# cahekp/Raymarching

Hardware: AMD Instinct MI355X
Metric: ray-steps/sec + frames/sec at 4096×4096, 1/2/4/8 MI355X (higher is better)
Workload: dtype f32; 1 GPU; C3: 4096x4096 scene T (template.frag), 256 max steps, pose P0, row bands of 16 over 1 GPU(s), rgba8 frame on rank 0; scene=T, W=4096, H=4096, max_steps=256, pose=P0, band=16, fmt=rgba8, wire=rgba8, streams=1, kernel=auto, chunks=1, schedule=adaptive, ray_steps_per_frame=1074511601, executed_ray_steps_per_frame=398047527

## Files before the change

include/rm.h:

```cpp
#ifndef RM_H_
#define RM_H_

#include <stddef.h>
#include <stdint.h>

#ifdef __cplusplus
extern "C" {
#endif

#define RM_ABI_VERSION 3

typedef enum rm_status {
    RM_OK = 0,
    RM_ERR_INVALID_ARGUMENT = 1,
    RM_ERR_FILE = 2,
    RM_ERR_SCENE = 3,
    RM_ERR_NO_SCENE = 4,
    RM_ERR_DEVICE = 5,
    RM_ERR_OUT_OF_MEMORY = 6
} rm_status;

typedef struct rm_ctx rm_ctx;

typedef struct rm_params {
// ... 170 lines not shown
    RM_TONEMAP_REINHARD = 2,
    RM_TONEMAP_REINHARD_JODIE = 3,
    RM_TONEMAP_UNCHARTED2 = 4
} rm_tonemap;

rm_status rm_post_frag(rm_ctx *ctx, int W, int H, int sample, int tonemap, const uint32_t *in, uint32_t *out);

rm_status rm_post_chain_ex(rm_ctx *ctx, int W, int H, int sample, int tonemap, const uint32_t *in, uint32_t *mid,
                           uint32_t *out);

rm_status rm_resolution_cache_info(rm_ctx *ctx, int *entries, int *capacity);

rm_status rm_certified_steps(rm_ctx *ctx, uint64_t *steps);

rm_status rm_reflection_cleared_steps(rm_ctx *ctx, uint64_t *steps);

const char *rm_render_code_hash(void);

rm_status rm_cycle_rows(int H, int cycle, int offset, int run, int *nrows);
rm_status rm_render_cycle_rows(rm_ctx *ctx, int W, int H, int cycle, int offset, int run, int row_begin,
                               int row_count, float *out, rm_stats *stats);
rm_status rm_render_cycle_rows_rgba8(rm_ctx *ctx, int W, int H, int cycle, int offset, int run, int row_begin,
                                     int row_count, uint32_t *out, rm_stats *stats);
rm_status rm_deinterleave_cycle_rgb8(rm_ctx *ctx, int W, int H, int cycle, int nparts, const int *offsets,
                                     const int *runs, const int64_t *part_bytes, const uint8_t *gathered,
                                     uint32_t *out);

int64_t rm_wire_capacity(int W, int nrows);
int64_t rm_wire_workspace_bytes(int W, int nrows);
rm_status rm_wire_encode(rm_ctx *ctx, int W, int nrows, const uint32_t *rows, uint8_t *msg, void *workspace,
// ... 41 lines not shown
```

raymarching_amd/_lib.py:

```python
from __future__ import annotations

import ctypes
import os

HERE = os.path.dirname(os.path.abspath(__file__))
LIB_PATH = os.environ.get("RM_LIB") or os.path.join(HERE, "librm.so")

RM_OK = 0
STATUS = {0: "RM_OK", 1: "RM_ERR_INVALID_ARGUMENT", 2: "RM_ERR_FILE", 3: "RM_ERR_SCENE",
          4: "RM_ERR_NO_SCENE", 5: "RM_ERR_DEVICE", 6: "RM_ERR_OUT_OF_MEMORY"}
STATUS_CODES = {v: k for k, v in STATUS.items()}

EXPORTS = ("rm_create", "rm_destroy", "rm_load_scene", "rm_set_uniform1f", "rm_set_uniform2f",
           "rm_set_uniform3f", "rm_set_params", "rm_get_params", "rm_set_stream", "rm_set_stream_kept",
           "rm_synchronize",
           "rm_render", "rm_render_band", "rm_render_rows", "rm_shard_rows", "rm_deinterleave", "rm_deinterleave_rgba8",
           "rm_pack_rgba8", "rm_pack_rgb8", "rm_deinterleave_rgb8",
           "rm_render_rgba8", "rm_render_accumulate", "rm_render_accumulate_rgba8", "rm_render_band_rgba8", "rm_render_rows_rgba8", "rm_fxaa", "rm_bloom", "rm_post_chain", "rm_post_frag", "rm_post_chain_ex",
           "rm_render_code_hash", "rm_render_cycle_rows_wire", "rm_last_error", "rm_status_string",
           "rm_compile_scene", "rm_scene_eval", "rm_render_step_map", "rm_sharded_layout", "rm_comm_get_id",
           "rm_comm_init_rank", "rm_comm_init_all", "rm_comm_destroy", "rm_render_sharded", "rm_render_sharded_all",
           "rm_set_tile_order", "rm_tile_grid", "rm_comm_info", "rm_abi_version", "rm_cycle_rows",
           "rm_render_cycle_rows", "rm_render_cycle_rows_rgba8", "rm_deinterleave_cycle_rgb8",
           "rm_render_sharded_runs", "rm_render_sharded_runs_all", "rm_wire_capacity", "rm_wire_workspace_bytes",
           "rm_wire_encode", "rm_wire_decode", "rm_scatter_part_rgba8", "rm_wire_decode_parts",
           "rm_set_uniform4f", "rm_set_uniform1i", "rm_set_uniformfv", "rm_uniform_count", "rm_uniform_info_at",
           "rm_get_uniformfv", "rm_get_uniform1i", "rm_cast_rays", "rm_camera_rays",
           "rm_aa_offsets", "rm_aa_edge_mask", "rm_refine_rgba8", "rm_render_aa_rgba8", "rm_shade_rays", "rm_scene_eval_form",
           "rm_resolution_cache_info", "rm_certified_steps", "rm_reflection_cleared_steps",
           "rm_batch_bytes", "rm_render_batch", "rm_render_batch_rgba8")

ABI_VERSION = 3
DISPATCH = {0: "row-major", 1: "explicit", 2: "adaptive"}
POST_SAMPLES = {"fxaa": 0, "texel": 1, "chromatic": 2}
TONEMAPS = {"none": 0, "aces": 1, "reinhard": 2, "jodie": 3, "uncharted2": 4}


class RmParams(ctypes.Structure):
    _fields_ = [("max_steps", ctypes.c_int32), ("shadow_max_steps", ctypes.c_int32),
                ("count_evals", ctypes.c_int32), ("kernel", ctypes.c_int32), ("schedule", ctypes.c_int32)]


class RmStats(ctypes.Structure):
    _fields_ = [("evals", ctypes.c_uint64), ("pixels", ctypes.c_uint64), ("kernel_ms", ctypes.c_float),
# ... 143 lines not shown
        "rm_sharded_layout": ([c.c_int, c.c_int, c.c_int, c.c_int, c.c_int, c.POINTER(RmShardLayout)], c.c_int),
        "rm_comm_get_id": ([c.POINTER(RmCommId)], c.c_int),
        "rm_comm_init_rank": ([c.POINTER(vp), vp, c.c_int, c.POINTER(RmCommId), c.c_int], c.c_int),
        "rm_comm_init_all": ([c.POINTER(vp), c.POINTER(vp), c.c_int], c.c_int),
        "rm_comm_destroy": ([vp], c.c_int),
        "rm_comm_info": ([vp, c.POINTER(c.c_int), c.POINTER(c.c_int), c.POINTER(c.c_int)], c.c_int),
        "rm_render_sharded": ([vp, c.c_int, c.c_int, c.c_int, vp, c.POINTER(RmStats)], c.c_int),
        "rm_render_sharded_all": ([c.POINTER(vp), c.c_int, c.c_int, c.c_int, c.c_int, vp, c.POINTER(RmStats)],
                                  c.c_int),
        "rm_set_tile_order": ([vp, vp, c.c_int64], c.c_int),
        "rm_tile_grid": ([c.POINTER(RmParams), c.c_int, c.c_int, c.POINTER(c.c_int), c.POINTER(c.c_int)], c.c_int),
        "rm_abi_version": ([], c.c_int),
        "rm_resolution_cache_info": ([vp, c.POINTER(c.c_int), c.POINTER(c.c_int)], c.c_int),
        "rm_certified_steps": ([vp, c.POINTER(c.c_uint64)], c.c_int),
        "rm_reflection_cleared_steps": ([vp, c.POINTER(c.c_uint64)], c.c_int),
        "rm_cycle_rows": ([c.c_int, c.c_int, c.c_int, c.c_int, c.POINTER(c.c_int)], c.c_int),
        "rm_render_cycle_rows": ([vp, c.c_int, c.c_int, c.c_int, c.c_int, c.c_int, c.c_int, c.c_int, vp,
                                  c.POINTER(RmStats)], c.c_int),
        "rm_render_cycle_rows_rgba8": ([vp, c.c_int, c.c_int, c.c_int, c.c_int, c.c_int, c.c_int, c.c_int, vp,
                                        c.POINTER(RmStats)], c.c_int),
        "rm_deinterleave_cycle_rgb8": ([vp, c.c_int, c.c_int, c.c_int, c.c_int, vp, vp, vp, vp, vp], c.c_int),
        "rm_wire_capacity": ([c.c_int, c.c_int], c.c_int64),
        "rm_wire_workspace_bytes": ([c.c_int, c.c_int], c.c_int64),
        "rm_wire_encode": ([vp, c.c_int, c.c_int, vp, vp, vp, vp], c.c_int),
        "rm_wire_decode": ([vp, c.c_int, c.c_int, c.c_int, c.c_int, c.c_int, c.c_int, vp, vp], c.c_int),
        "rm_scatter_part_rgba8": ([vp, c.c_int, c.c_int, c.c_int, c.c_int, c.c_int, c.c_int, vp, vp], c.c_int),
        "rm_wire_decode_parts": ([vp, c.c_int, c.c_int, c.c_int, c.c_int, vp, vp, vp, vp, vp], c.c_int),
        "rm_render_sharded_runs": ([vp, c.c_int, c.c_int, vp, vp, c.POINTER(RmStats)], c.c_int),
        "rm_render_sharded_runs_all": ([c.POINTER(vp), c.c_int, c.c_int, c.c_int, vp, vp, c.POINTER(RmStats)],
                                       c.c_int),
# ... 19 lines not shown
```

raymarching_amd/api.py:

```python
from __future__ import annotations

import ctypes
import sys

from . import _lib
from ._lib import RmParams, RmStats, check, lib


def _torch():
    import torch
    return torch


class Renderer:

    def __init__(self, device: int = 0):
        L = lib()
        self._ctx = ctypes.c_void_p()
        st = L.rm_create(ctypes.byref(self._ctx), int(device))
        if st != 0:
            raise _lib.RmError(st, f"rm_create(device={device}) failed")
        self.device = int(device)
        self._uniform_types = {}

# ... 123 lines not shown

    @staticmethod
    def _ptr(t):
        return ctypes.c_void_p(t.data_ptr()) if hasattr(t, "data_ptr") else ctypes.c_void_p(t.ctypes.data)

    def certified_steps(self) -> int:
        n = ctypes.c_uint64(0)
        check(lib().rm_certified_steps(self._ctx, ctypes.byref(n)), self._ctx)
        return int(n.value)

    def reflection_cleared_steps(self) -> int:
        n = ctypes.c_uint64(0)
        check(lib().rm_reflection_cleared_steps(self._ctx, ctypes.byref(n)), self._ctx)
        return int(n.value)

    def _stats(self, s) -> dict:
        return dict(s.as_dict(), certified=self.certified_steps(), reflection_cleared=self.reflection_cleared_steps())

    def render(self, W: int, H: int, out=None, stats: bool = False):
        torch = _torch()
        if out is None:
            out = torch.empty((H, W, 4), dtype=torch.float32, device=f"cuda:{self.device}")
        _check_out(out, H * W * 4)
        s = RmStats()
        check(lib().rm_render(self._ctx, int(W), int(H), self._ptr(out), ctypes.byref(s) if stats else None),
              self._ctx)
        return (out, self._stats(s)) if stats else out

    def render_accumulate(self, W: int, H: int, accum, stats: bool = False):
        torch = _torch()
        rgba8 = accum.dtype == torch.int32
        if not rgba8 and accum.dtype != torch.float32:
# ... 635 lines not shown
```

raymarching_amd/csrc/rm_batch_host.cpp:

```cpp
#include <cmath>
#include <cstring>

#include "rm_batch.h"
#include "rm_ctx.h"
#include "rm_trace.h"

using rm::FrameConst;
using rm::RowPart;
using namespace rmhost;

namespace {

int64_t pixel_bytes(bool rgba8) { return rgba8 ? (int64_t)sizeof(uint32_t) : (int64_t)sizeof(float4); }

rm_status batch_host_block(rm_ctx *ctx, size_t bytes, rm_ctx::BatchSlot *&slot) {
    slot = &ctx->batch_slot[ctx->batch_next];
    ctx->batch_next = (ctx->batch_next + 1) % rm_ctx::kBatchSlots;
    if (slot->used) RM_HIP(hipEventSynchronize(slot->copied));
    slot->used = false;
    if (!slot->copied) RM_HIP(hipEventCreateWithFlags(&slot->copied, hipEventDisableTiming));
    if (slot->bytes < bytes) {
        if (slot->host) (void)hipHostFree(slot->host);
        slot->host = nullptr;
        slot->bytes = 0;
// ... 22 lines not shown
    if (rm_status st = frame_rcp(ctx, F)) return st;
    F.row0 = 0;
    F.tile_run = rm::wave_row_mode(part, 0, 8, F.run_magic != 0);
    F.lat_tiles = 0;

    const size_t bytes = (size_t)n * rm::batch_record_bytes(ctx->scene);
    rm_ctx::BatchSlot *slot = nullptr;
    if (rm_status st = batch_host_block(ctx, bytes, slot)) return st;
    FrameConst V = F;
    for (int v = 0; v < n; v++) {
        pose_const(V, views[v].pos, views[v].mouse, views[v].time);
        V.jit_x = seed_jitter(views[v].offset[0] + 0.5f);
        V.jit_y = seed_jitter(views[v].offset[1] + 0.5f);
        rm::batch_record_write(ctx->scene, slot->host, v, V);
    }
    if (rm_status st = batch_scratch(ctx, bytes)) return st;
    void *rec_d = ctx->batch_views;
    RM_HIP(hipMemcpyAsync(rec_d, slot->host, bytes, hipMemcpyHostToDevice, ctx->stream));
    RM_HIP(hipEventRecord(slot->copied, ctx->stream));
    slot->used = true;
    ctx->batch_stream = ctx->stream;
    ctx->batch_pending = true;
    mark_done(ctx);

    ctx->last_certified = 0;
    ctx->last_refl_cleared = 0;
    if (stats) RM_HIP(hipEventRecord(ctx->ev0, ctx->stream));
    const hipError_t e = ctx->scene == rm::SCENE_S0 || ctx->scene == rm::SCENE_T
                             ? rm::launch_batch_t(ctx->scene, F, rec_d, n, out, rgba8, ctx->stream)
                             : rm::launch_batch_o(ctx->scene, F, rec_d, n, out, rgba8, ctx->stream);
    if (e != hipSuccess) return hip_fail(ctx, e, "view batch launch");
    if (stats) {
        RM_HIP(hipEventRecord(ctx->ev1, ctx->stream));
        RM_HIP(hipEventSynchronize(ctx->ev1));
        float ms = 0.0f;
        RM_HIP(hipEventElapsedTime(&ms, ctx->ev0, ctx->ev1));
        std::memset(stats, 0, sizeof(*stats));
        stats->pixels = (uint64_t)n * (uint64_t)W * (uint64_t)H;
        stats->kernel_ms = ms;
        stats->scene = ctx->scene;
        stats->dispatch = RM_DISPATCH_ROW_MAJOR;
// ... 60 lines not shown
```

raymarching_amd/csrc/rm_capi.cpp:

```cpp
#include <cstdio>
#include <cstring>
#include <fstream>
#include <initializer_list>
#include <string>

#include "rm_ctx.h"
#include "rm_internal.h"
#include "rm_scene_file.h"
#include "rm_trace.h"

using rm::cycle_part;
using rm::FrameConst;
using rm::RowPart;
using rm::rows_of_part;
using namespace rmhost;

static_assert(rmscene::kSceneS0 == rm::SCENE_S0 && rmscene::kSceneT == rm::SCENE_T &&
                  rmscene::kSceneO == rm::SCENE_O && rmscene::kSceneOG == rm::SCENE_OG &&
                  rmscene::kScenePlugin == rm::SCENE_PLUGIN,
              "rm_scene_file.h restates rm::SceneId");

namespace {

template <class Launch>
// ... 24 lines not shown
void rm_internal_set_error(rm_ctx *ctx, const std::string &msg) { ctx->err = msg; }

extern "C" {

rm_status rm_create(rm_ctx **out, int device) {
    if (!out) return RM_ERR_INVALID_ARGUMENT;
    *out = nullptr;
    int n = 0;
    if (hipGetDeviceCount(&n) != hipSuccess || device < 0 || device >= n) {
        (void)hipGetLastError();
        return RM_ERR_DEVICE;
    }
    rm_ctx *ctx = new rm_ctx();
    ctx->device = device;
    hipError_t e = hipSetDevice(device);
    if (e == hipSuccess) e = hipMalloc(&ctx->d_evals, 5 * sizeof(unsigned long long));
    if (e == hipSuccess) e = hipEventCreate(&ctx->ev0);
    if (e == hipSuccess) e = hipEventCreate(&ctx->ev1);
    if (e == hipSuccess) e = hipEventCreateWithFlags(&ctx->done, hipEventDisableTiming);
    ctx->persist.reserve(rm_ctx::kPersistBlocks);
    if (e != hipSuccess) {
        rm_destroy(ctx);
        return e == hipErrorOutOfMemory ? RM_ERR_OUT_OF_MEMORY : RM_ERR_DEVICE;
    }
    *out = ctx;
    return RM_OK;
}

rm_status rm_destroy(rm_ctx *ctx) {
    if (!ctx) return RM_ERR_INVALID_ARGUMENT;
    (void)hipSetDevice(ctx->device);
// ... 739 lines not shown

int rm_abi_version(void) { return RM_ABI_VERSION; }

rm_status rm_certified_steps(rm_ctx *ctx, uint64_t *steps) {
    if (!ctx || !steps) return RM_ERR_INVALID_ARGUMENT;
    *steps = ctx->last_certified;
    return RM_OK;
}

rm_status rm_reflection_cleared_steps(rm_ctx *ctx, uint64_t *steps) {
    if (!ctx || !steps) return RM_ERR_INVALID_ARGUMENT;
    *steps = ctx->last_refl_cleared;
    return RM_OK;
}

rm_status rm_resolution_cache_info(rm_ctx *ctx, int *entries, int *capacity) {
    if (!ctx) return RM_ERR_INVALID_ARGUMENT;
    if (entries) *entries = ctx->rcp_n;
    if (capacity) *capacity = rm_ctx::kRcpEntries;
    return RM_OK;
}

const char *rm_last_error(rm_ctx *ctx) { return ctx ? ctx->err.c_str() : "null context"; }

const char *rm_status_string(rm_status s) {
    switch (s) {
    case RM_OK: return "RM_OK";
    case RM_ERR_INVALID_ARGUMENT: return "RM_ERR_INVALID_ARGUMENT";
    case RM_ERR_FILE: return "RM_ERR_FILE";
    case RM_ERR_SCENE: return "RM_ERR_SCENE";
// ... 9 lines not shown
```

raymarching_amd/csrc/rm_ctx.h:

```cpp
#pragma once
#include <hip/hip_runtime.h>

#include <set>
#include <string>
#include <vector>

#include "../../include/rm.h"
#include "rm_launch.h"
#include "rm_plugin_host.h"
#include "rm_rows.h"

struct rm_ctx {
    int device = 0;
    hipStream_t stream = nullptr;
    int scene = -1;
    std::string scene_file;
    float res[2] = {0.0f, 0.0f};
    bool res_set = false;
    float pos[3] = {0.0f, 0.0f, 0.0f};
    float mouse[2] = {0.0f, 0.0f};
    float time = 0.0f;
    struct PersistBlock {
        hipStream_t stream = nullptr;
        uint32_t *ctr = nullptr;
// ... 1 lines not shown
        uint64_t used = 0;
    };
    static constexpr int kPersistBlocks = 4;
    std::vector<PersistBlock> persist;
    hipEvent_t done = nullptr;
    bool dirty = false;
    std::vector<hipEvent_t> retired;
    std::vector<hipStream_t> kept, owed;
    float sample_part = 1.0f;
    float seed1[2] = {0.0f, 0.0f}, seed2[2] = {0.0f, 0.0f};
    rm_params params = {128, 0, 0, 0, 1};
    std::string err;
    std::set<std::string> warned;
    unsigned long long *d_evals = nullptr;
    unsigned long long last_certified = 0;
    unsigned long long last_refl_cleared = 0;
    hipEvent_t ev0 = nullptr, ev1 = nullptr;
    float4 *staging = nullptr;
    size_t staging_bytes = 0;
    uint32_t *mips = nullptr;
    size_t mips_texels = 0;
    int bloom_runs_w = 0, bloom_runs_h = 0;
    hipStream_t bloom_runs_stream = nullptr;
    hipEvent_t bloom_ev = nullptr;
    hipStream_t bloom_stream = nullptr;
    bool bloom_pending = false;
    uint32_t *aa_queue = nullptr;
    size_t aa_words = 0;
    hipEvent_t aa_ev = nullptr;
    hipStream_t aa_stream = nullptr;
// ... 115 lines not shown
```

raymarching_amd/csrc/rm_device.h:

```cpp
#pragma once
#ifdef __HIPCC_RTC__
using __hip_internal::uint32_t;
using __hip_internal::uint64_t;
#else
#include <hip/hip_runtime.h>
#include <stdint.h>
#endif
#include "rm_far_sky.h"
#include "rm_shadow_clear.h"
#include "rm_refl_clear.h"

namespace rm {

enum SceneId : int { SCENE_S0 = 0, SCENE_T = 1, SCENE_O = 2, SCENE_OG = 3, SCENE_PLUGIN = 4 };

constexpr float ZNEAR = 0.02f;
constexpr float ZFAR = 50.0f;
constexpr float PI_REF = 3.1416f;

struct FrameConst {
    float res_x, res_y;
    float pos_x, pos_y, pos_z;
    float cam1_c, cam1_s;
    float cam2_c, cam2_s;
// ... 10 lines not shown
    float sss_floor[2][32];
    uint32_t* evals_map;
    const uint32_t* tile_order;
    uint32_t* tile_cost;
    int lat_tiles;
    int accumulate;
    float sample_part;
    float jit_x, jit_y;
    uint32_t* persist;
    uint32_t run_magic;
    uint32_t gx_magic;
    float camq_x, camq_y, camq_z;
    int far_sky;
    float rcp_w, rcp_h, rcp_res_y;
    int tile_run;
};
static_assert(rmfs::kFarSkyDepth == ZFAR, "rm_far_sky.h restates ZFAR");
static_assert(rmrc::kNear == ZNEAR, "rm_refl_clear.h restates ZNEAR");

__host__ inline void camera_sponge_origin(FrameConst& F) {
    const float x = F.pos_x, y = F.pos_y - 3.0f, z = F.pos_z;
    const float x1 = __builtin_fmaf(x, F.ry_c, z * F.ry_s);
    const float z1 = __builtin_fmaf(z, F.ry_c, -(x * F.ry_s));
    F.camq_x = x1;
    F.camq_y = __builtin_fmaf(y, F.rx_c, -(z1 * F.rx_s));
    F.camq_z = __builtin_fmaf(z1, F.rx_c, y * F.rx_s);
}

__host__ __device__ inline uint32_t div_magic(uint32_t d, uint64_t a_end) {
    return d >= 2 && a_end * (uint64_t)d < (1ull << 32) ? (uint32_t)((1ull << 32) / d + 1) : 0u;
// ... 78 lines not shown
    const float c1 = y2 * (y2 * (y2 * -0.0204391631f + 0.2536086171f) + -1.2336977925f) + 1.0f;
    const float s1 = y * (y2 * (y2 * (y2 * -0.0046075748f + 0.0796819754f) + -0.645963615f) + 1.5707963235f);
    const float c2 = c1 * c1 - s1 * s1;
    const float s2 = 2.0f * s1 * c1;
    return 2.0f * s2 * c2 * (1.0f / (s2 * s2 + c2 * c2));
}
__host__ __device__ inline float glsl_cos(float x) { return glsl_sin(x + 1.57079632f); }


struct Tally {
    uint32_t evals = 0;
    uint32_t flop = 0;
    uint32_t skipped = 0;
    uint32_t certified = 0;
    uint32_t refl_cleared = 0;
};
constexpr uint32_t FL_SPHERE = 9;
constexpr uint32_t FL_TRANSFORM = 18;
constexpr uint32_t FL_LINRAY = 6;
constexpr uint32_t FL_BOX = 17;
constexpr uint32_t FL_FOLD = 40;
constexpr uint32_t FL_CUBE = 21;
constexpr uint32_t FL_SMIN = 12;
constexpr uint32_t FL_BOUNDS = 16;

__device__ __forceinline__ float div_const(float x, float b, float rb) {
    float q = x * rb;
    float r = fmaf(-b, q, x);
    return fmaf(r, rb, q);
}
// ... 299 lines not shown
```

raymarching_amd/csrc/rm_far_sky.h:

```cpp
#pragma once

#if defined(__HIPCC__) || defined(__HIPCC_RTC__) || defined(__HIP__)
#define RM_FS_HD __host__ __device__
#else
#define RM_FS_HD
#endif

namespace rmfs {

constexpr float kFarSkyM = 0.25f;
constexpr float kFarSkyR = 1.0f + kFarSkyM + 0x1p-10f;
constexpr int kFarSkyN0 = 208;
constexpr float kFarSkyFar = 4.1f;
constexpr float kFarSkyDepth = 50.0f;

RM_FS_HD inline bool ray_misses_cube(float ox, float oy, float oz, float dx, float dy, float dz, float r) {
    const float ax = __builtin_fabsf(ox), ay = __builtin_fabsf(oy), az = __builtin_fabsf(oz);
    const float bx = __builtin_fabsf(dx), by = __builtin_fabsf(dy), bz = __builtin_fabsf(dz);
    const float sxy = bx + by, syz = by + bz, szx = bz + bx;
    const bool ok = (ax + ay + az <= 1024.0f) & (sxy + bz <= 4.0f);
    const float tiny = 0x1p-100f;
    const bool cz = __builtin_fabsf(__builtin_fmaf(ox, dy, -(oy * dx))) > __builtin_fmaf(r, sxy, tiny);
    const bool cx = __builtin_fabsf(__builtin_fmaf(oy, dz, -(oz * dy))) > __builtin_fmaf(r, syz, tiny);
    const bool cy = __builtin_fabsf(__builtin_fmaf(oz, dx, -(ox * dz))) > __builtin_fmaf(r, szx, tiny);
// ... 3 lines not shown
    return ok & (cx | cy | cz | fx | fy | fz);
}

RM_FS_HD inline bool far_point_clear(float ox, float oy, float oz, float dx, float dy, float dz) {
    const float qx = __builtin_fmaf(dx, kFarSkyDepth, ox), qy = __builtin_fmaf(dy, kFarSkyDepth, oy);
    const float qz = __builtin_fmaf(dz, kFarSkyDepth, oz);
    return __builtin_fmaxf(__builtin_fabsf(qx), __builtin_fmaxf(__builtin_fabsf(qy), __builtin_fabsf(qz))) >= kFarSkyFar;
}

RM_FS_HD inline bool far_sky_ray(float ox, float oy, float oz, float dx, float dy, float dz) {
    const bool miss = ray_misses_cube(ox, oy, oz, dx, dy, dz, kFarSkyR);
    const bool clear = far_point_clear(ox, oy, oz, dx, dy, dz);
    return miss & clear;
}

}
```

raymarching_amd/csrc/rm_rays_host.cpp:

```cpp
#include <cstring>

#include "rm_ctx.h"
#include "rm_rays.h"
#include "rm_trace.h"

using rm::FrameConst;
using rm::RowPart;
using namespace rmhost;

static_assert((int)RM_RAY_MISS == (int)rm::RAY_MISS && (int)RM_RAY_HIT == (int)rm::RAY_HIT &&
                  (int)RM_RAY_EXHAUSTED == (int)rm::RAY_EXHAUSTED,
              "rm.h RM_RAY_* and rm_rays.h RAY_*");

namespace {

constexpr int64_t kMaxRays = (int64_t)1 << 30;

rm_status cast_dev(rm_ctx *ctx, rm::RayQuery Q, int inside, rm_stats *stats) {
    rm::TraceRange range("rm_cast_rays");
    const FrameConst F = frame_const(ctx, 1, 1, RowPart{1, 0, 1}, 1);
    if (stats) {
        Q.evals = ctx->d_evals;
        RM_HIP(hipMemsetAsync(ctx->d_evals, 0, 5 * sizeof(unsigned long long), ctx->stream));
        RM_HIP(hipEventRecord(ctx->ev0, ctx->stream));
    }
    const hipError_t e =
        ctx->scene == rm::SCENE_PLUGIN
            ? rmplugin::launch_cast(ctx->plugin, F, ctx->uniform_values, Q, inside, rm::cast_block_size(), ctx->stream)
            : rm::launch_cast_rays(ctx->scene, F, Q, inside, ctx->stream);
    if (e != hipSuccess) return hip_fail(ctx, e, "cast kernel launch");
    mark_done(ctx);
    if (stats) {
        RM_HIP(hipEventRecord(ctx->ev1, ctx->stream));
        RM_HIP(hipEventSynchronize(ctx->ev1));
        float ms = 0.0f;
        RM_HIP(hipEventElapsedTime(&ms, ctx->ev0, ctx->ev1));
        unsigned long long ev = 0;
        RM_HIP(hipMemcpy(&ev, ctx->d_evals, sizeof(ev), hipMemcpyDeviceToHost));
        std::memset(stats, 0, sizeof(*stats));
        stats->evals = ev;
        ctx->last_certified = 0;
        ctx->last_refl_cleared = 0;
        stats->pixels = (uint64_t)Q.n;
        stats->kernel_ms = ms;
        stats->scene = ctx->scene;
    }
    return RM_OK;
}

}

extern "C" {

rm_status rm_cast_rays(rm_ctx *ctx, const float *origins, int shared_origin, const float *directions, int64_t n,
                       int inside, const rm_ray_hits *out, rm_stats *stats) {
    if (!ctx) return RM_ERR_INVALID_ARGUMENT;
    if (n < 0 || n > kMaxRays || (n > 0 && (!origins || !directions || !out || !out->t)))
// ... 108 lines not shown
```

raymarching_amd/csrc/rm_render_direct.h:

```cpp
#pragma once
#include "rm_device.h"
#include "rm_wire_tile.h"

namespace rm {

__device__ __forceinline__ V3 cnormalize(V3 a) { return a * __builtin_amdgcn_rsqf(dot(a, a)); }
template <int SC, int NB = 3>
__device__ __forceinline__ float dist_march(const FrameConst& F, V3 p, Tally& cnt) {
    return scene_dist<SC, ScenePolicy<SC>::kExactMarch, NB>(F, p, cnt);
}
template <int SC, int NB = 3>
__device__ __forceinline__ float dist_probe(const FrameConst& F, V3 p, Tally& cnt) {
    return scene_dist<SC, kProbeForm, NB>(F, p, cnt);
}
template <int SC>
__device__ __forceinline__ V3 mnormalize(V3 a) {
    if constexpr (ScenePolicy<SC>::kHwMath) return a * __builtin_amdgcn_rsqf(dot(a, a));
    else return normalize(a);
}

__device__ __forceinline__ float plane_rate(V3 d) {
    return __builtin_amdgcn_rcpf(1.01f + fabsf(d.y));
}
template <int SC>
// ... 446 lines not shown
    }
    if constexpr (SC == SCENE_OG || SC == SCENE_PLUGIN) {
        if (m.transparency > 0.0f) {
            V3 r = refract(rd, n, 1.0f / m.refraction_index);
            color = color + (render_refraction<SC, SETTLE>(F, p + r * 0.001f, r, m.absorption, cnt) * (1.0f - rf)) *
                                m.transparency;
        }
    }
    return color;
}

template <int NB = 3, int SETTLE = 0, int RSTOP = 0>
__device__ __forceinline__ V3 render_T_from(const FrameConst& F, const LinRay& prim, V3 ro, V3 rd, Tally& cnt) {
    constexpr int SC = SCENE_T;
    using P = ScenePolicy<SC>;
    bool far = false;
    if constexpr (P::kFarSky && RSTOP != 0) {
        if (F.far_sky)
            far = __builtin_amdgcn_ballot_w64(
                      rmfs::far_sky_ray(prim.o.x, prim.o.y, prim.o.z, prim.d.x, prim.d.y, prim.d.z)) ==
                  __builtin_amdgcn_ballot_w64(true);
    }
    const uint32_t e0 = cnt.evals;
    float depth = ZFAR;
    if (RSTOP != 1 || !far) depth = cast_ray_T<NB>(F, prim, cnt);
    if constexpr (RSTOP == 2) cnt.skipped += far ? cnt.evals - e0 : 0u;
    V3 p = ro + rd * depth;
    const bool boxp = RSTOP == 1 && far;
    V3 n;
    if (boxp) n = normal_fast<SC, NB, true>(F, p, cnt);
    else n = normal_fast<SC, NB>(F, p, cnt);
    float c = 1.0f;
    if (RSTOP != 1 || !far) {
        const uint32_t e1 = cnt.evals, s1 = cnt.skipped;
        V3 rdir = reflect(rd, n);
        V3 ror = p + rdir * 0.01f;
        const LinRay rray = sponge_ray(F, ror, rdir);
        bool rclear = false;
        if constexpr (P::kReflClear && RSTOP != 0)
            rclear = (F.max_steps >= rmrc::kSteps) &
                     rmrc::refl_clear(rray.o.x, rray.o.y, rray.o.z, rray.d.x, rray.d.y, rray.d.z);
        if (RSTOP != 1 || !rclear) {
            V3 pr = ror + rdir * cast_ray_T<NB, RSTOP>(F, rray, cnt);
            if constexpr (RSTOP == 2) {
                cnt.skipped = far ? s1 + (cnt.evals - e1) : cnt.skipped;
                Tally none;
                const bool phit = menger_at<NB>(prim, depth, none) < 0.001f;
                cnt.refl_cleared += rclear && phit ? (cnt.evals - e1) - (cnt.skipped - s1) : 0u;
            }
            const V3 pd = pr - p;
            c = clamp01_as<P::kTrim>(__builtin_amdgcn_sqrtf(dot(pd, pd)) * (1.0f / 3.0f));
        }
        (void)e1; (void)s1;
    }
    (void)e0;
    const V3 lightPos = v3(20.0f, 50.0f, 0.0f);
    V3 Ld = lightPos - p;
    float ld2 = dot(Ld, Ld);
    V3 lightDir = Ld * __builtin_amdgcn_rsqf(ld2);
    float occ;
    if (boxp) occ = ao_real<SC, NB, true>(F, p, n, cnt);
    else occ = ao_real<SC, NB>(F, p, n, cnt);
    const LinRay sray = sponge_ray(F, p, lightDir);
// ... 117 lines not shown

__device__ __forceinline__ uint32_t wave_sum_u32(uint32_t v) {
#pragma unroll
    for (int o = 32; o > 0; o >>= 1) v += __shfl_xor(v, o, 64);
    return v;
}

__device__ __forceinline__ uint32_t tile_clocks(uint64_t t_start) {
    const uint64_t dt = clock64() - t_start;
    return dt > 0xffffffffull ? 0xffffffffu : (uint32_t)dt;
}
__device__ __forceinline__ void store_tally(const FrameConst& F, unsigned long long* evals, const Tally& cnt, int x,
                                            int j, int lane) {
    if (F.evals_map && x < F.W && j < F.nrows) F.evals_map[(size_t)j * F.W + x] = cnt.evals;
    uint32_t se = wave_sum_u32(cnt.evals), sf = wave_sum_u32(cnt.flop), ss = wave_sum_u32(cnt.skipped);
    uint32_t sc = wave_sum_u32(cnt.certified), sr = wave_sum_u32(cnt.refl_cleared);
    if (lane == 0) {
        atomicAdd(&evals[0], (unsigned long long)se);
        atomicAdd(&evals[1], (unsigned long long)sf);
        if (ss) atomicAdd(&evals[2], (unsigned long long)ss);
        if (sc) atomicAdd(&evals[3], (unsigned long long)sc);
        if (sr) atomicAdd(&evals[4], (unsigned long long)sr);
    }
}

template <int SC, int NB = 3, int SETTLE = 0, int RSTOP = 0>
__device__ __forceinline__ V3 render_pixel(const FrameConst& F, V3 ro, V3 rd, Tally& cnt) {
    if constexpr (SC == SCENE_S0) return render_S0(F, ro, rd, cnt);
    else if constexpr (SC == SCENE_T) return render_T<NB, SETTLE, RSTOP>(F, ro, rd, cnt);
    else return render_O<SC, SETTLE>(F, ro, rd, cnt);
}

template <int SC, int FORM = kFormExact>
__device__ __forceinline__ void scene_eval_one(const FrameConst& F, const float* pts, long long n, float* dist,
                                               float* mat, float* aux = nullptr) {
    const long long i = (long long)blockIdx.x * blockDim.x + threadIdx.x;
    if (i >= n) return;
// ... 111 lines not shown
```

raymarching_amd/csrc/rm_render_host.cpp:

```cpp
#include <algorithm>
#include <cmath>
#include <cstring>

#include "rm_ctx.h"
#include "rm_trace.h"

using rm::FrameConst;
using rm::RowPart;

namespace rmhost {
namespace {

inline float fract(float x) { return x - std::floor(x); }

float hash11(float p) {
    float a = fract(p * 443.897f);
    float x = a, y = a, z = a;
    float dd = x * (y + 19.19f) + y * (z + 19.19f) + z * (x + 19.19f);
    x += dd; y += dd; z += dd;
    return fract((x + y) * z);
}

float sss_floor_term(float ny, int i) {
    const float fi = (float)i, nx = -0.0f, nyn = -ny, nz = -0.0f;
// ... 26 lines not shown
    if (ctx->staging) (void)hipFree(ctx->staging);
    ctx->staging = nullptr;
    ctx->staging_bytes = 0;
    RM_HIP(hipMalloc(&ctx->staging, bytes));
    ctx->staging_bytes = bytes;
    return RM_OK;
}

int pick_kernel(const rm_params &p) {
    if (p.kernel == 1) return rm::KERNEL_TILE16;
    if (p.kernel == 3) return rm::KERNEL_TILE16X4;
    if (p.kernel == 4) return rm::KERNEL_PERSIST;
    return rm::KERNEL_TILE8;
}

void pose_const(FrameConst &F, const float pos[3], const float mouse[2], float time) {
    F.pos_x = pos[0]; F.pos_y = pos[1]; F.pos_z = pos[2];
    float a1 = -mouse[1], a2 = mouse[0];
    F.cam1_c = rm::glsl_cos(a1); F.cam1_s = rm::glsl_sin(a1);
    F.cam2_c = rm::glsl_cos(a2); F.cam2_s = rm::glsl_sin(a2);
    float rot_y = time * 2.0f, rot_x = 180.0f;
    float ay = -rot_y * 0.017453292519943295f, ax = -rot_x * 0.017453292519943295f;
    F.ry_c = rm::glsl_cos(ay); F.ry_s = rm::glsl_sin(ay);
    F.rx_c = rm::glsl_cos(ax); F.rx_s = rm::glsl_sin(ax);
    rm::camera_sponge_origin(F);
    F.time = time;
    F.mouse_x = mouse[0];
    F.mouse_y = mouse[1];
}

float seed_jitter(float seed) { return (seed - std::floor(seed)) - 0.5f; }

FrameConst frame_const(const rm_ctx *c, int W, int H, const RowPart &part, int nrows) {
    FrameConst F;
    std::memset(&F, 0, sizeof(F));
    F.res_x = c->res_set ? c->res[0] : (float)W;
    F.res_y = c->res_set ? c->res[1] : (float)H;
    pose_const(F, c->pos, c->mouse, c->time);
    F.W = W; F.H = H;
    F.cycle = part.cycle; F.offset = part.offset; F.run = part.run; F.nrows = nrows;
    F.run_magic = rm::div_magic((uint32_t)part.run, (uint64_t)H + 1);
    F.max_steps = c->params.max_steps;
    F.shadow_max_steps = c->params.shadow_max_steps > 0 ? c->params.shadow_max_steps : 0x7fffffff;
    F.far_sky = c->scene == rm::SCENE_T && F.max_steps >= rmfs::kFarSkyN0 ? 1 : 0;
    F.lat_tiles = lat_tiles_for(pick_kernel(c->params), W, nrows);
    for (int i = 0; i < 32; i++) {
        F.hash11[i] = hash11((float)i);
        F.sss_floor[0][i] = sss_floor_term(1.0f, i);
        F.sss_floor[1][i] = sss_floor_term(0x1.fffffep-1f, i);
    }
    return F;
}

rm_status frame_rcp(rm_ctx *ctx, FrameConst &F) {
    if (ctx->scene != rm::SCENE_S0 && ctx->scene != rm::SCENE_T) return RM_OK;
    uint32_t bits;
    std::memcpy(&bits, &F.res_y, sizeof(bits));
// ... 49 lines not shown
                F.tile_cost = sc->buf + ((k / P) & 1) * sc->n;
            if (k >= 1) {
                const uint64_t s = (k - 1) / P;
                F.tile_order = sc->buf + (2 + (s & 1)) * sc->n;
            }
        }
    }
    rm_ctx::PersistBlock *pb = nullptr;
    if (ctx->scene != rm::SCENE_PLUGIN && kernel == rm::KERNEL_PERSIST) {
        rm_status st = persist_block(ctx, pb);
        if (st != RM_OK) return st;
        F.persist = pb->ctr;
    }
    ctx->last_certified = 0;
    ctx->last_refl_cleared = 0;
    bool cnt = ctx->params.count_evals != 0 || evmap;
    if (cnt) RM_HIP(hipMemsetAsync(ctx->d_evals, 0, 5 * sizeof(unsigned long long), ctx->stream));
    if (stats) RM_HIP(hipEventRecord(ctx->ev0, ctx->stream));
    hipError_t e =
        wire ? rm::launch_render_wire(ctx->scene, F, static_cast<rm::WireTile *>(out), cnt ? ctx->d_evals : nullptr,
                                      ctx->stream)
        : ctx->scene == rm::SCENE_PLUGIN
            ? rmplugin::launch_render(ctx->plugin, F, ctx->uniform_values, out, rgba8, cnt ? ctx->d_evals : nullptr, ctx->stream)
            : rm::launch_render(ctx->scene, F, out, rgba8, cnt ? ctx->d_evals : nullptr, kernel, ctx->stream);
    if (e != hipSuccess) return hip_fail(ctx, e, "render kernel launch");
    if (stats) RM_HIP(hipEventRecord(ctx->ev1, ctx->stream));
    if (wire) {
        e = rm::launch_wire_finish(out, W, count, wire->msg, wire->size_out, ctx->stream);
        if (e != hipSuccess) return hip_fail(ctx, e, "wire scan/compact launch");
    }
    if (pb) RM_HIP(hipEventRecord(pb->last, ctx->stream));
    if (sc && F.tile_cost) {
// ... 1 lines not shown
        uint32_t *h = sc->buf + 4 * (size_t)sc->n;
        e = rm::launch_tile_order(sc->buf + slot * sc->n, sc->n, sc->gx, kSchedDilate, sc->buf + (2 + slot) * sc->n,
                                  h + 512 * slot, h + 512 * (1 - slot), reinterpret_cast<uint8_t *>(h + 1024),
                                  ctx->stream);
        if (e != hipSuccess) return hip_fail(ctx, e, "tile order launch");
    }
    if (sc) {
        sc->dirty = true;
        if (!cnt) sc->k++;
    }
    mark_done(ctx);
    if (stats) {
        RM_HIP(hipEventSynchronize(ctx->ev1));
        float ms = 0.0f;
        RM_HIP(hipEventElapsedTime(&ms, ctx->ev0, ctx->ev1));
        unsigned long long ev[5] = {0, 0, 0, 0, 0};
        if (cnt) RM_HIP(hipMemcpy(ev, ctx->d_evals, sizeof(ev), hipMemcpyDeviceToHost));
        std::memset(stats, 0, sizeof(*stats));
        stats->evals = ev[0];
        stats->flop = ev[1];
        stats->skipped = ev[2];
        ctx->last_certified = ev[3];
        ctx->last_refl_cleared = ev[4];
        stats->pixels = (uint64_t)W * (uint64_t)count;
        stats->kernel_ms = ms;
        stats->scene = ctx->scene;
        stats->dispatch = !F.tile_order ? RM_DISPATCH_ROW_MAJOR
                          : F.tile_order == ctx->tile_order ? RM_DISPATCH_EXPLICIT
                                                            : RM_DISPATCH_ADAPTIVE;
        if (F.tile_order && ctx->scene == rm::SCENE_T && kernel != rm::KERNEL_TILE16) {
            const rm::TileGrid g = rm::tile_grid(kernel, W, count);
            stats->lat_tiles = std::min(F.lat_tiles, g.x * g.y);
        }
    }
    return RM_OK;
}

rm_status render_part(rm_ctx *ctx, int W, int H, const RowPart &part, int row_begin, int row_count, void *out,
// ... 49 lines not shown
```

raymarching_amd/csrc/rm_shade_host.cpp:

```cpp
#include <cstring>

#include "rm_ctx.h"
#include "rm_shade.h"
#include "rm_trace.h"

using rm::FrameConst;
using rm::RowPart;
using namespace rmhost;

namespace {

constexpr int64_t kMaxRays = (int64_t)1 << 30;

rm_status shade_dev(rm_ctx *ctx, const FrameConst &F, const rm::ShadeRays &Q, rm_stats *stats) {
    rm::TraceRange range("rm_shade_rays");
    if (stats) RM_HIP(hipEventRecord(ctx->ev0, ctx->stream));
    const hipError_t e = ctx->scene == rm::SCENE_PLUGIN
                             ? rmplugin::launch_shade(ctx->plugin, F, ctx->uniform_values, Q, ctx->stream)
                         : ctx->scene == rm::SCENE_S0 || ctx->scene == rm::SCENE_T
                             ? rm::launch_shade_rays_t(ctx->scene, F, Q, ctx->stream)
                             : rm::launch_shade_rays_o(ctx->scene, F, Q, ctx->stream);
    if (e != hipSuccess) return hip_fail(ctx, e, "shade kernel launch");
    mark_done(ctx);
    if (stats) {
        RM_HIP(hipEventRecord(ctx->ev1, ctx->stream));
        RM_HIP(hipEventSynchronize(ctx->ev1));
        float ms = 0.0f;
        RM_HIP(hipEventElapsedTime(&ms, ctx->ev0, ctx->ev1));
        std::memset(stats, 0, sizeof(*stats));
        stats->pixels = (uint64_t)Q.n;
        ctx->last_certified = 0;
        ctx->last_refl_cleared = 0;
        stats->kernel_ms = ms;
        stats->scene = ctx->scene;
    }
    return RM_OK;
}

}

extern "C" {

rm_status rm_shade_rays(rm_ctx *ctx, const float *origins, int shared_origin, const float *directions, int64_t n,
                        const rm_shade_params *params, float *out_rgba, uint32_t *out_rgba8, rm_stats *stats) {
    if (!ctx) return RM_ERR_INVALID_ARGUMENT;
    if (n < 0 || n > kMaxRays || (n > 0 && (!params || !origins || !directions)) ||
        (out_rgba != nullptr) == (out_rgba8 != nullptr))
// ... 90 lines not shown
```

Measured before the change: 4695 billion ray-steps/s.

## Add near-sky bounding-cube early-out with step-budget ladder for scene T

Adds a ladder of tighter bounding-cube radii, each certified by a constexpr step bound. Waves whose rays all miss the tighter cube and whose far point is clear skip the march when RSTOP is 1. The radius is chosen from max_steps, and the code falls back to the far-sky cube when the camera rotations are not unit. With RSTOP==2 the vote only counts near-sky steps for diagnostics, and a sixth counter slot and API accessor are added. The goal is to skip marching for more sky rays at 256 steps. The cost is an extra per-ray cube test, and correctness rests on the proven step bounds.

```diff
diff --git a/include/rm.h b/include/rm.h
--- a/include/rm.h
+++ b/include/rm.h
@@ -208,6 +208,8 @@
 rm_status rm_certified_steps(rm_ctx *ctx, uint64_t *steps);
 
 rm_status rm_reflection_cleared_steps(rm_ctx *ctx, uint64_t *steps);
+
+rm_status rm_near_sky_steps(rm_ctx *ctx, uint64_t *steps);
 
 const char *rm_render_code_hash(void);
 
diff --git a/raymarching_amd/_lib.py b/raymarching_amd/_lib.py
--- a/raymarching_amd/_lib.py
+++ b/raymarching_amd/_lib.py
@@ -28,6 +28,7 @@
            "rm_get_uniformfv", "rm_get_uniform1i", "rm_cast_rays", "rm_camera_rays",
            "rm_aa_offsets", "rm_aa_edge_mask", "rm_refine_rgba8", "rm_render_aa_rgba8", "rm_shade_rays", "rm_scene_eval_form",
            "rm_resolution_cache_info", "rm_certified_steps", "rm_reflection_cleared_steps",
+           "rm_near_sky_steps",
            "rm_batch_bytes", "rm_render_batch", "rm_render_batch_rgba8")
 
 ABI_VERSION = 3
@@ -201,6 +202,7 @@
         "rm_resolution_cache_info": ([vp, c.POINTER(c.c_int), c.POINTER(c.c_int)], c.c_int),
         "rm_certified_steps": ([vp, c.POINTER(c.c_uint64)], c.c_int),
         "rm_reflection_cleared_steps": ([vp, c.POINTER(c.c_uint64)], c.c_int),
+        "rm_near_sky_steps": ([vp, c.POINTER(c.c_uint64)], c.c_int),
         "rm_cycle_rows": ([c.c_int, c.c_int, c.c_int, c.c_int, c.POINTER(c.c_int)], c.c_int),
         "rm_render_cycle_rows": ([vp, c.c_int, c.c_int, c.c_int, c.c_int, c.c_int, c.c_int, c.c_int, vp,
                                   c.POINTER(RmStats)], c.c_int),
diff --git a/raymarching_amd/api.py b/raymarching_amd/api.py
--- a/raymarching_amd/api.py
+++ b/raymarching_amd/api.py
@@ -161,8 +161,14 @@
         check(lib().rm_reflection_cleared_steps(self._ctx, ctypes.byref(n)), self._ctx)
         return int(n.value)
 
+    def near_sky_steps(self) -> int:
+        n = ctypes.c_uint64(0)
+        check(lib().rm_near_sky_steps(self._ctx, ctypes.byref(n)), self._ctx)
+        return int(n.value)
+
     def _stats(self, s) -> dict:
-        return dict(s.as_dict(), certified=self.certified_steps(), reflection_cleared=self.reflection_cleared_steps())
+        return dict(s.as_dict(), certified=self.certified_steps(), reflection_cleared=self.reflection_cleared_steps(),
+                    near_sky=self.near_sky_steps())
 
     def render(self, W: int, H: int, out=None, stats: bool = False):
         torch = _torch()
diff --git a/raymarching_amd/csrc/rm_batch_host.cpp b/raymarching_amd/csrc/rm_batch_host.cpp
--- a/raymarching_amd/csrc/rm_batch_host.cpp
+++ b/raymarching_amd/csrc/rm_batch_host.cpp
@@ -60,6 +60,7 @@
         V.jit_y = seed_jitter(views[v].offset[1] + 0.5f);
         rm::batch_record_write(ctx->scene, slot->host, v, V);
     }
+    F.near_r = V.near_r;
     if (rm_status st = batch_scratch(ctx, bytes)) return st;
     void *rec_d = ctx->batch_views;
     RM_HIP(hipMemcpyAsync(rec_d, slot->host, bytes, hipMemcpyHostToDevice, ctx->stream));
@@ -71,6 +72,7 @@
 
     ctx->last_certified = 0;
     ctx->last_refl_cleared = 0;
+    ctx->last_near_sky = 0;
     if (stats) RM_HIP(hipEventRecord(ctx->ev0, ctx->stream));
     const hipError_t e = ctx->scene == rm::SCENE_S0 || ctx->scene == rm::SCENE_T
                              ? rm::launch_batch_t(ctx->scene, F, rec_d, n, out, rgba8, ctx->stream)
diff --git a/raymarching_amd/csrc/rm_capi.cpp b/raymarching_amd/csrc/rm_capi.cpp
--- a/raymarching_amd/csrc/rm_capi.cpp
+++ b/raymarching_amd/csrc/rm_capi.cpp
@@ -62,7 +62,7 @@
     rm_ctx *ctx = new rm_ctx();
     ctx->device = device;
     hipError_t e = hipSetDevice(device);
-    if (e == hipSuccess) e = hipMalloc(&ctx->d_evals, 5 * sizeof(unsigned long long));
+    if (e == hipSuccess) e = hipMalloc(&ctx->d_evals, 6 * sizeof(unsigned long long));
     if (e == hipSuccess) e = hipEventCreate(&ctx->ev0);
     if (e == hipSuccess) e = hipEventCreate(&ctx->ev1);
     if (e == hipSuccess) e = hipEventCreateWithFlags(&ctx->done, hipEventDisableTiming);
@@ -832,6 +832,12 @@
     return RM_OK;
 }
 
+rm_status rm_near_sky_steps(rm_ctx *ctx, uint64_t *steps) {
+    if (!ctx || !steps) return RM_ERR_INVALID_ARGUMENT;
+    *steps = ctx->last_near_sky;
+    return RM_OK;
+}
+
 rm_status rm_resolution_cache_info(rm_ctx *ctx, int *entries, int *capacity) {
     if (!ctx) return RM_ERR_INVALID_ARGUMENT;
     if (entries) *entries = ctx->rcp_n;
diff --git a/raymarching_amd/csrc/rm_ctx.h b/raymarching_amd/csrc/rm_ctx.h
--- a/raymarching_amd/csrc/rm_ctx.h
+++ b/raymarching_amd/csrc/rm_ctx.h
@@ -39,6 +39,7 @@
     std::set<std::string> warned;
     unsigned long long *d_evals = nullptr;
     unsigned long long last_certified = 0;
+    unsigned long long last_near_sky = 0;
     unsigned long long last_refl_cleared = 0;
     hipEvent_t ev0 = nullptr, ev1 = nullptr;
     float4 *staging = nullptr;
diff --git a/raymarching_amd/csrc/rm_device.h b/raymarching_amd/csrc/rm_device.h
--- a/raymarching_amd/csrc/rm_device.h
+++ b/raymarching_amd/csrc/rm_device.h
@@ -48,6 +48,7 @@
     int far_sky;
     float rcp_w, rcp_h, rcp_res_y;
     int tile_run;
+    float near_r;
 };
 static_assert(rmfs::kFarSkyDepth == ZFAR, "rm_far_sky.h restates ZFAR");
 static_assert(rmrc::kNear == ZNEAR, "rm_refl_clear.h restates ZNEAR");
@@ -156,6 +157,7 @@
     uint32_t skipped = 0;
     uint32_t certified = 0;
     uint32_t refl_cleared = 0;
+    uint32_t near_sky = 0;
 };
 constexpr uint32_t FL_SPHERE = 9;
 constexpr uint32_t FL_TRANSFORM = 18;
diff --git a/raymarching_amd/csrc/rm_far_sky.h b/raymarching_amd/csrc/rm_far_sky.h
--- a/raymarching_amd/csrc/rm_far_sky.h
+++ b/raymarching_amd/csrc/rm_far_sky.h
@@ -41,4 +41,61 @@
     return miss & clear;
 }
 
+
+constexpr double kUnitLo = 0.999, kUnitHi = 1.001;
+constexpr float kUnitRotTol = 1.0e-4f;
+
+constexpr int near_sky_bound(float r) {
+    const double m = (double)r - 1.0 - 0x1p-10, e = 0x1p-12;
+    const double s3lo = 1.7320508075, s3hi = 1.7320508076;
+    const double c = kUnitLo / s3hi, vmin = s3lo * m;
+    if (!(m >= 0.015625)) return 0x7fffffff;
+    int nA = 0;
+    for (double v = 1025.0; v > vmin; v *= 1.0 - c) nA++;
+    const int nB = (int)(2.0 * s3hi * (1.0 + e + m) / (kUnitLo * m)) + 1;
+    int nC = 0;
+    for (double g = 1.0; (g - 1.0) * vmin < 50.0 * kUnitHi; g *= 1.0 + c) nC++;
+    return nA + nB + nC;
 }
+
+struct NearSkyRung {
+    float m;
+    float r;
+    int n;
+};
+constexpr NearSkyRung near_sky_rung(float m) {
+    const float r = 1.0f + m + 0x1p-10f;
+    return NearSkyRung{m, r, near_sky_bound(r)};
+}
+constexpr int kNearSkyRungs = 4;
+constexpr NearSkyRung kNearSkyLadder[kNearSkyRungs] = {near_sky_rung(0.25f), near_sky_rung(0.1f), near_sky_rung(0.05f),
+                                                       near_sky_rung(0.02f)};
+static_assert(kNearSkyLadder[0].r == kFarSkyR && kNearSkyLadder[0].n <= kFarSkyN0, "the first rung is the far-sky cube");
+static_assert(kNearSkyLadder[0].n < kNearSkyLadder[1].n && kNearSkyLadder[1].n < kNearSkyLadder[2].n &&
+                  kNearSkyLadder[2].n < kNearSkyLadder[3].n,
+              "a smaller m needs more steps");
+static_assert(kNearSkyLadder[2].n <= 128 && kNearSkyLadder[3].n <= kFarSkyN0, "m = 0.05 under 128 steps, m = 0.02 under N0");
+
+inline bool unit_rotation(float c, float s) {
+    const float n = c * c + s * s - 1.0f;
+    return n <= kUnitRotTol && n >= -kUnitRotTol;
+}
+
+inline float near_sky_radius(int max_steps, bool unit_dirs) {
+    float r = 0.0f;
+    if (unit_dirs) {
+        for (int i = 0; i < kNearSkyRungs; i++)
+            if (max_steps >= kNearSkyLadder[i].n) r = kNearSkyLadder[i].r;
+    } else if (max_steps >= kFarSkyN0) {
+        r = kFarSkyR;
+    }
+    return r;
+}
+
+RM_FS_HD inline bool near_sky_ray(float ox, float oy, float oz, float dx, float dy, float dz, float r) {
+    const bool miss = ray_misses_cube(ox, oy, oz, dx, dy, dz, r);
+    const bool clear = far_point_clear(ox, oy, oz, dx, dy, dz);
+    return miss & clear;
+}
+
+}
diff --git a/raymarching_amd/csrc/rm_rays_host.cpp b/raymarching_amd/csrc/rm_rays_host.cpp
--- a/raymarching_amd/csrc/rm_rays_host.cpp
+++ b/raymarching_amd/csrc/rm_rays_host.cpp
@@ -21,7 +21,7 @@
     const FrameConst F = frame_const(ctx, 1, 1, RowPart{1, 0, 1}, 1);
     if (stats) {
         Q.evals = ctx->d_evals;
-        RM_HIP(hipMemsetAsync(ctx->d_evals, 0, 5 * sizeof(unsigned long long), ctx->stream));
+        RM_HIP(hipMemsetAsync(ctx->d_evals, 0, 6 * sizeof(unsigned long long), ctx->stream));
         RM_HIP(hipEventRecord(ctx->ev0, ctx->stream));
     }
     const hipError_t e =
@@ -41,6 +41,7 @@
         stats->evals = ev;
         ctx->last_certified = 0;
         ctx->last_refl_cleared = 0;
+        ctx->last_near_sky = 0;
         stats->pixels = (uint64_t)Q.n;
         stats->kernel_ms = ms;
         stats->scene = ctx->scene;
diff --git a/raymarching_amd/csrc/rm_render_direct.h b/raymarching_amd/csrc/rm_render_direct.h
--- a/raymarching_amd/csrc/rm_render_direct.h
+++ b/raymarching_amd/csrc/rm_render_direct.h
@@ -484,17 +484,32 @@
 __device__ __forceinline__ V3 render_T_from(const FrameConst& F, const LinRay& prim, V3 ro, V3 rd, Tally& cnt) {
     constexpr int SC = SCENE_T;
     using P = ScenePolicy<SC>;
-    bool far = false;
+    bool far = false, vote = false;
     if constexpr (P::kFarSky && RSTOP != 0) {
-        if (F.far_sky)
-            far = __builtin_amdgcn_ballot_w64(
-                      rmfs::far_sky_ray(prim.o.x, prim.o.y, prim.o.z, prim.d.x, prim.d.y, prim.d.z)) ==
+        if (F.near_r > 0.0f) {
+            float r = F.near_r;
+            asm volatile("" : "+v"(r));
+            vote = __builtin_amdgcn_ballot_w64(
+                      rmfs::near_sky_ray(prim.o.x, prim.o.y, prim.o.z, prim.d.x, prim.d.y, prim.d.z, r)) ==
                   __builtin_amdgcn_ballot_w64(true);
-    }
+        }
+        if constexpr (RSTOP == 2) {
+            if (F.far_sky)
+                far = __builtin_amdgcn_ballot_w64(
+                          rmfs::far_sky_ray(prim.o.x, prim.o.y, prim.o.z, prim.d.x, prim.d.y, prim.d.z)) ==
+                      __builtin_amdgcn_ballot_w64(true);
+        } else {
+            far = vote;
+        }
+    }
+    const bool near = RSTOP == 2 && vote && !far;
     const uint32_t e0 = cnt.evals;
     float depth = ZFAR;
     if (RSTOP != 1 || !far) depth = cast_ray_T<NB>(F, prim, cnt);
-    if constexpr (RSTOP == 2) cnt.skipped += far ? cnt.evals - e0 : 0u;
+    if constexpr (RSTOP == 2) {
+        cnt.skipped += far ? cnt.evals - e0 : 0u;
+        cnt.near_sky += near ? cnt.evals - e0 : 0u;
+    }
     V3 p = ro + rd * depth;
     const bool boxp = RSTOP == 1 && far;
     V3 n;
@@ -517,6 +532,7 @@
                 Tally none;
                 const bool phit = menger_at<NB>(prim, depth, none) < 0.001f;
                 cnt.refl_cleared += rclear && phit ? (cnt.evals - e1) - (cnt.skipped - s1) : 0u;
+                cnt.near_sky += near ? (cnt.evals - e1) - (cnt.skipped - s1) : 0u;
             }
             const V3 pd = pr - p;
             c = clamp01_as<P::kTrim>(__builtin_amdgcn_sqrtf(dot(pd, pd)) * (1.0f / 3.0f));
@@ -664,13 +680,14 @@
                                             int j, int lane) {
     if (F.evals_map && x < F.W && j < F.nrows) F.evals_map[(size_t)j * F.W + x] = cnt.evals;
     uint32_t se = wave_sum_u32(cnt.evals), sf = wave_sum_u32(cnt.flop), ss = wave_sum_u32(cnt.skipped);
-    uint32_t sc = wave_sum_u32(cnt.certified), sr = wave_sum_u32(cnt.refl_cleared);
+    uint32_t sc = wave_sum_u32(cnt.certified), sr = wave_sum_u32(cnt.refl_cleared), sn = wave_sum_u32(cnt.near_sky);
     if (lane == 0) {
         atomicAdd(&evals[0], (unsigned long long)se);
         atomicAdd(&evals[1], (unsigned long long)sf);
         if (ss) atomicAdd(&evals[2], (unsigned long long)ss);
         if (sc) atomicAdd(&evals[3], (unsigned long long)sc);
         if (sr) atomicAdd(&evals[4], (unsigned long long)sr);
+        if (sn) atomicAdd(&evals[5], (unsigned long long)sn);
     }
 }
 
diff --git a/raymarching_amd/csrc/rm_render_host.cpp b/raymarching_amd/csrc/rm_render_host.cpp
--- a/raymarching_amd/csrc/rm_render_host.cpp
+++ b/raymarching_amd/csrc/rm_render_host.cpp
@@ -64,6 +64,11 @@
     return rm::KERNEL_TILE8;
 }
 
+static bool pose_keeps_unit(const FrameConst &F) {
+    return rmfs::unit_rotation(F.cam1_c, F.cam1_s) && rmfs::unit_rotation(F.cam2_c, F.cam2_s) &&
+           rmfs::unit_rotation(F.ry_c, F.ry_s) && rmfs::unit_rotation(F.rx_c, F.rx_s);
+}
+
 void pose_const(FrameConst &F, const float pos[3], const float mouse[2], float time) {
     F.pos_x = pos[0]; F.pos_y = pos[1]; F.pos_z = pos[2];
     float a1 = -mouse[1], a2 = mouse[0];
@@ -74,6 +79,7 @@
     F.ry_c = rm::glsl_cos(ay); F.ry_s = rm::glsl_sin(ay);
     F.rx_c = rm::glsl_cos(ax); F.rx_s = rm::glsl_sin(ax);
     rm::camera_sponge_origin(F);
+    if (F.near_r > 0.0f && !pose_keeps_unit(F)) F.near_r = rmfs::near_sky_radius(F.max_steps, false);
     F.time = time;
     F.mouse_x = mouse[0];
     F.mouse_y = mouse[1];
@@ -86,11 +92,12 @@
     std::memset(&F, 0, sizeof(F));
     F.res_x = c->res_set ? c->res[0] : (float)W;
     F.res_y = c->res_set ? c->res[1] : (float)H;
+    F.max_steps = c->params.max_steps;
+    F.near_r = c->scene == rm::SCENE_T ? rmfs::near_sky_radius(F.max_steps, true) : 0.0f;
     pose_const(F, c->pos, c->mouse, c->time);
     F.W = W; F.H = H;
     F.cycle = part.cycle; F.offset = part.offset; F.run = part.run; F.nrows = nrows;
     F.run_magic = rm::div_magic((uint32_t)part.run, (uint64_t)H + 1);
-    F.max_steps = c->params.max_steps;
     F.shadow_max_steps = c->params.shadow_max_steps > 0 ? c->params.shadow_max_steps : 0x7fffffff;
     F.far_sky = c->scene == rm::SCENE_T && F.max_steps >= rmfs::kFarSkyN0 ? 1 : 0;
     F.lat_tiles = lat_tiles_for(pick_kernel(c->params), W, nrows);
@@ -170,8 +177,9 @@
     }
     ctx->last_certified = 0;
     ctx->last_refl_cleared = 0;
+    ctx->last_near_sky = 0;
     bool cnt = ctx->params.count_evals != 0 || evmap;
-    if (cnt) RM_HIP(hipMemsetAsync(ctx->d_evals, 0, 5 * sizeof(unsigned long long), ctx->stream));
+    if (cnt) RM_HIP(hipMemsetAsync(ctx->d_evals, 0, 6 * sizeof(unsigned long long), ctx->stream));
     if (stats) RM_HIP(hipEventRecord(ctx->ev0, ctx->stream));
     hipError_t e =
         wire ? rm::launch_render_wire(ctx->scene, F, static_cast<rm::WireTile *>(out), cnt ? ctx->d_evals : nullptr,
@@ -203,7 +211,7 @@
         RM_HIP(hipEventSynchronize(ctx->ev1));
         float ms = 0.0f;
         RM_HIP(hipEventElapsedTime(&ms, ctx->ev0, ctx->ev1));
-        unsigned long long ev[5] = {0, 0, 0, 0, 0};
+        unsigned long long ev[6] = {0, 0, 0, 0, 0, 0};
         if (cnt) RM_HIP(hipMemcpy(ev, ctx->d_evals, sizeof(ev), hipMemcpyDeviceToHost));
         std::memset(stats, 0, sizeof(*stats));
         stats->evals = ev[0];
@@ -211,6 +219,7 @@
         stats->skipped = ev[2];
         ctx->last_certified = ev[3];
         ctx->last_refl_cleared = ev[4];
+        ctx->last_near_sky = ev[5];
         stats->pixels = (uint64_t)W * (uint64_t)count;
         stats->kernel_ms = ms;
         stats->scene = ctx->scene;
diff --git a/raymarching_amd/csrc/rm_shade_host.cpp b/raymarching_amd/csrc/rm_shade_host.cpp
--- a/raymarching_amd/csrc/rm_shade_host.cpp
+++ b/raymarching_amd/csrc/rm_shade_host.cpp
@@ -31,6 +31,7 @@
         stats->pixels = (uint64_t)Q.n;
         ctx->last_certified = 0;
         ctx->last_refl_cleared = 0;
+        ctx->last_near_sky = 0;
         stats->kernel_ms = ms;
         stats->scene = ctx->scene;
     }
```

After: 4914 billion ray-steps/s (median of 6 runs). 1.05x the previous value.
